# GinZhu/RDST

Hardware: AMD Instinct MI355X
Metric: SR patches/sec fwd+bwd, RDST-E1 x4 64->256 (higher is better)
Workload: dtype bf16; 1 GPU; RDST-E1 x4 (RDST_E1_OASIS_example_SRx4.ini), 1x64x64 LR patches -> 256x256, step = fwd + L1 + bwd + flat-bucket grad all-reduce + Adam; global_batch=32, per_gpu_batch=32, parallelism=dp1, hip_graph=True, grad_bucket_bytes=17859844

## Files before the change

### rdst_amd/csrc/lnlin3_mfma.hip

```cpp
#include "linear.h"
#include "lds_dma.h"
#include "mfma.h"
#include "wattn_hd.h"
#include <stdlib.h>

#ifndef LB3_LOADW_SHAPE
#define LB3_LOADW_SHAPE(K, N) (((K) == 60 && (N) == 180) || ((K) == 90 && (N) == 270) || ((K) == 120 && (N) == 120))
#endif
#ifndef LB3_ABL
#define LB3_ABL 0
#endif

#ifdef LB3_STAMPS
constexpr bool LB3_TICKS = true;
#else
constexpr bool LB3_TICKS = false;
#endif
constexpr const char* LB3_LEGEND = "stash fetch barrier compute finish - - -";

namespace {
using namespace wahd;
using MM = Mma<bf16>;

struct LB3Args {
  const bf16* X; int64_t ldx; const float* stats; const float* lnw; const float* W;
  const bf16* dY; int64_t lddy; bf16* dX; int64_t lddx; const bf16* Acc; int64_t ldacc;
  const bf16* Acc2; int64_t ldacc2;
  float* slab; int64_t slab_stride;
  int64_t M; int64_t ntiles; int tiles_per_wg;
};

template <int K_, int N_>
struct LB3 {
  static constexpr int K = K_, N = N_;
  static constexpr int NCT = (K + 1 + 31) / 32, NW = (N + 31) / 32, KN = (N + 15) / 16;
  static constexpr bool WIDE = N >= 180;
  static constexpr int TN = WIDE ? 3 : 1;
  static constexpr int TC = (K == 120 && N == 360) ? 2 : WIDE ? 1 : NCT;
  static_assert(NW % TN == 0 && NCT % TC == 0, "blocking");
  static constexpr int NGN = NW / TN, NGC = NCT / TC, NWG = NGN * NGC;
  static constexpr int NDG = NCT;
  static constexpr int NWV = NWG + NDG, NT = 64 * NWV;
  static constexpr int PKX = (K * 2 + 15) / 16, PKY = (N * 2 + 15) / 16;
  static constexpr int NY = 32 * PKY, NX = 32 * PKX;
  static constexpr bool LOADW = LB3_LOADW_SHAPE(K_, N_);
  static constexpr bool SPLITR = WIDE || LOADW;
  static constexpr int NTW = SPLITR ? 64 * NWG : NT, NTD = SPLITR ? 64 * NDG : NT;
  static constexpr int cdiv(int a, int b) { return (a + b - 1) / b; }
  static constexpr bool ACC_BY_W = K == 120 && N == 360;
  static constexpr int W_SY = cdiv(NY, NTW), W_SX = cdiv(NX, NTW), W_SA = (WIDE && !ACC_BY_W && !LOADW) ? 0 : cdiv(NX, NTW);
  static constexpr int D_SY = SPLITR ? 0 : W_SY, D_SX = SPLITR ? 0 : W_SX, D_SA = (ACC_BY_W || LOADW) ? 0 : cdiv(NX, NTD);
  static constexpr int CP = 32 * NCT;
  static constexpr int LDX = NCT == 4 ? 336 : CP * 2 + 16;
  static constexpr int LDY = lds_plane_stride(32 * NW);
  static constexpr int OFF_AC = 32 * LDX, OFF_DY = 64 * LDX, OFF_SM = OFF_DY + 32 * LDY, BUF = OFF_SM + 128;
  static constexpr int OFF_RED = 2 * BUF;
  static constexpr int SMEM = OFF_RED + 2 * NCT * 256;
  static constexpr int PERCU0 = 12 / NWV < 1 ? 1 : 12 / NWV;
  static constexpr int PERCU1 = WIDE ? 1 : PERCU0 > 2 ? 2 : PERCU0;
  static constexpr int PERCU = PERCU1 * SMEM > 160 * 1024 ? 1 : PERCU1;
  static constexpr int WPS = (NWV * PERCU + 3) / 4;
};

template <class CF, bool LN, int SY, int SX, int SA>
struct LB3Loader {
  static constexpr int NS = SY + SX + SA;
  int meta[NS > 0 ? NS : 1];
  u32x4_a4 rd[NS > 0 ? NS : 1];
  u32x4_a4 rd2[SA > 0 ? SA : 1];
  float2 rst[SX > 0 ? SX : 1];
  static __device__ __forceinline__ int kind(int u) { return u < SY ? 0 : u < SY + SX ? 1 : 2; }
  __device__ __forceinline__ void setup(int tid_r, int ntr, bool has_acc) {
#pragma unroll
    for (int u = 0; u < NS; ++u) {
      const int kd = kind(u);
      const int idx = tid_r + ntr * (kd == 0 ? u : kd == 1 ? u - SY : u - SY - SX);
      const int per = kd == 0 ? CF::PKY : CF::PKX, rowbytes = kd == 0 ? CF::N * 2 : CF::K * 2;
      const bool on = idx < 32 * per && (kd != 2 || has_acc);
      const int row = on ? idx / per : 0, chk = on ? idx - row * per : 0;
      int o = chk * 16;
      if (o + 16 > rowbytes) o = rowbytes - 16;
      meta[u] = o | (row << 16) | ((on ? 1 : 0) << 24) | (((o & 15) == 0 ? 1 : 0) << 28);
    }
  }
  __device__ __forceinline__ void fetch(const LB3Args& p, int64_t tile) {
    const uint32_t Mu = (uint32_t)p.M;
#pragma unroll
    for (int u = 0; u < NS; ++u) {
      const int kd = kind(u);
      uint32_t row = (uint32_t)(tile * 32) + (uint32_t)((meta[u] >> 16) & 31);
      row = row < Mu ? row : Mu - 1;
      const char* base = reinterpret_cast<const char*>(kd == 0 ? p.dY : kd == 1 ? p.X : (p.Acc ? p.Acc : p.X));
      const uint32_t ldb = (uint32_t)((kd == 0 ? p.lddy : kd == 1 ? p.ldx : p.ldacc) * 2);
      rd[u] = *reinterpret_cast<const u32x4_a4*>(base + (size_t)(row * ldb + (uint32_t)(meta[u] & 0xffff)));
      if (kd == 2 && p.Acc2)
        rd2[u - SY - SX] = *reinterpret_cast<const u32x4_a4*>(reinterpret_cast<const char*>(p.Acc2) +
                                                              (size_t)(row * (uint32_t)(p.ldacc2 * 2) + (uint32_t)(meta[u] & 0xffff)));
      if (LN && kd == 1) rst[u - SY] = *reinterpret_cast<const float2*>(p.stats + 2 * (size_t)row);
    }
  }
  __device__ __forceinline__ void stash(const LB3Args& p, int64_t tile, char* buf) {
    const uint32_t Mu = (uint32_t)p.M;
#pragma unroll
    for (int u = 0; u < NS; ++u) {
      const int kd = kind(u);
      if (!((meta[u] >> 24) & 1)) continue;
      const int mrow = (meta[u] >> 16) & 31;
      const bool valid = (uint32_t)(tile * 32) + (uint32_t)mrow < Mu;
      Pack16 v;
      v.w[0] = valid ? rd[u].x : 0u; v.w[1] = valid ? rd[u].y : 0u; v.w[2] = valid ? rd[u].z : 0u; v.w[3] = valid ? rd[u].w : 0u;
      if (kd == 2 && p.Acc2) {
        const u32x4_a4 a = rd[u], b2 = rd2[u - SY - SX];
        const bool h1 = p.Acc != nullptr;
        float f[8];
        f[0] = bf16lo(b2.x) + (h1 ? bf16lo(a.x) : 0.f); f[1] = bf16hi(b2.x) + (h1 ? bf16hi(a.x) : 0.f);
        f[2] = bf16lo(b2.y) + (h1 ? bf16lo(a.y) : 0.f); f[3] = bf16hi(b2.y) + (h1 ? bf16hi(a.y) : 0.f);
        f[4] = bf16lo(b2.z) + (h1 ? bf16lo(a.z) : 0.f); f[5] = bf16hi(b2.z) + (h1 ? bf16hi(a.z) : 0.f);
        f[6] = bf16lo(b2.w) + (h1 ? bf16lo(a.w) : 0.f); f[7] = bf16hi(b2.w) + (h1 ? bf16hi(a.w) : 0.f);
#pragma unroll
        for (int e = 0; e < 8; ++e) f[e] = valid ? f[e] : 0.f;
        v = MM::pack(f);
      }
      if (LN && kd == 1) {
        const float2 st2 = rst[u - SY];
        float f[8];
        f[0] = bf16lo(rd[u].x); f[1] = bf16hi(rd[u].x); f[2] = bf16lo(rd[u].y); f[3] = bf16hi(rd[u].y);
        f[4] = bf16lo(rd[u].z); f[5] = bf16hi(rd[u].z); f[6] = bf16lo(rd[u].w); f[7] = bf16hi(rd[u].w);
#pragma unroll
        for (int e = 0; e < 8; ++e) f[e] = valid ? (f[e] - st2.x) * st2.y : 0.f;
        v = MM::pack(f);
        if ((meta[u] & 0xffff) == 0) reinterpret_cast<float*>(buf + CF::OFF_SM)[mrow] = st2.y;
      }
      int mt = meta[u];
      asm volatile("" : "+v"(mt));
      const int lrow = (mt >> 16) & 31, lo = mt & 0xffff;
      char* dst = buf + (kd == 0 ? CF::OFF_DY + lrow * CF::LDY : (kd == 2 ? CF::OFF_AC : 0) + lrow * CF::LDX) + lo;
      if ((meta[u] >> 28) & 1) *reinterpret_cast<Pack16*>(dst) = v;
      else {
        uint32_t* d = reinterpret_cast<uint32_t*>(dst);
        d[0] = v.w[0]; d[1] = v.w[1]; d[2] = v.w[2]; d[3] = v.w[3];
      }
    }
  }
};

template <int K, int N, bool LN>
__global__ void __launch_bounds__((LB3<K, N>::NT), (LB3<K, N>::WPS)) lnlin3_bwd_kernel(const LB3Args p) {
  extern __shared__ __attribute__((aligned(16))) char smem[];
  using CF = LB3<K, N>;
  constexpr int NCT = CF::NCT, NW = CF::NW, KN = CF::KN, TN = CF::TN, TC = CF::TC, NGC = CF::NGC, NWG = CF::NWG, NT = CF::NT;
  constexpr int LDX = CF::LDX, LDY = CF::LDY;
  const int tid = threadIdx.x, lane = tid & 63, wave = __builtin_amdgcn_readfirstlane(tid >> 6), r = lane & 31, hh = lane >> 5;
  const bool has_acc = p.Acc != nullptr || p.Acc2 != nullptr;

  if (!(LB3_ABL & 16)) lds_zero16(smem, CF::SMEM, tid, NT);
  __syncthreads();
  if (tid < 64) *reinterpret_cast<uint16_t*>(smem + (tid >> 5) * CF::BUF + (tid & 31) * LDX + K * 2) = 0x3f80;

  const int q = (lane & 15) >> 2, pp = lane & 3, gq1 = (lane >> 4) & 1;
  const int trc = (16 * gq1 + 4 * pp) * 2;
  const int tro_y = CF::OFF_DY + (8 * hh + q) * LDY + trc;
  const int tro_x = (8 * hh + q) * LDX + trc;

  const bool is_wg = wave < NWG;
  const int gn = wave / NGC, gc = wave - gn * NGC;
  const int dct = wave - NWG;

  const int64_t t0 = (int64_t)blockIdx.x * p.tiles_per_wg;
  const int64_t t1 = t0 + p.tiles_per_wg < p.ntiles ? t0 + p.tiles_per_wg : p.ntiles;
  __syncthreads();

  if (is_wg) {
    LB3Loader<CF, LN, CF::W_SY, CF::W_SX, CF::W_SA> ld;
    ld.setup(tid, CF::NTW, has_acc);
    if (t0 < t1) ld.fetch(p, t0);
    f32x16 G[TN][TC];
#pragma unroll
    for (int i = 0; i < TN; ++i)
#pragma unroll
      for (int j = 0; j < TC; ++j)
#pragma unroll
        for (int v = 0; v < 16; ++v) G[i][j][v] = 0.f;
    int b = 0;
    WaveTicks<LB3_TICKS> wt;
    for (int64_t tile = t0; tile < t1; ++tile, b ^= 1) {
      char* buf = smem + b * CF::BUF;
      ld.stash(p, tile, buf);
      wt.add(0);
      ld.fetch(p, tile + 1 < t1 ? tile + 1 : tile);
      wt.add(1);
      __syncthreads();
      wt.add(2);
#pragma unroll
      for (int s = 0; s < 2; ++s) {
        Pack16 ya[TN], xb[TC];
#pragma unroll
        for (int i = 0; i < TN; ++i) {
          const lds_cp yp = (lds_cp)(buf + tro_y + 16 * s * LDY) + (gn * TN + i) * 64;
          ya[i] = lds_tr_pack(yp, yp + 4 * LDY);
        }
#pragma unroll
        for (int j = 0; j < TC; ++j) {
          const lds_cp xp = (lds_cp)(buf + tro_x + 16 * s * LDX) + (gc * TC + j) * 64;
          xb[j] = lds_tr_pack(xp, xp + 4 * LDX);
        }
#pragma unroll
        for (int i = 0; i < TN; ++i)
#pragma unroll
          for (int j = 0; j < TC; ++j) {
#if !(LB3_ABL & 1)
            MM::mma(G[i][j], ya[i], xb[j]);
#else
            G[i][j][0] += __uint_as_float(ya[i].w[0] ^ xb[j].w[0]);
#endif
          }
      }
      wt.add(3);
    }
    wt.print(wave, lane, "wgrad", LB3_LEGEND);
    if (LN) __syncthreads();
    uint2* my = reinterpret_cast<uint2*>(p.slab) + (int64_t)blockIdx.x * p.slab_stride;
#pragma unroll
    for (int i = 0; i < TN; ++i)
#pragma unroll
      for (int j = 0; j < TC; ++j) {
        const int c = 32 * (gc * TC + j) + r;
#pragma unroll
        for (int g4 = 0; g4 < 4; ++g4) {
          const int n0 = 32 * (gn * TN + i) + 8 * g4 + 4 * hh;
          if (n0 < N && c <= K && !(LB3_ABL & 8))
            my[(int64_t)(n0 >> 2) * (K + 1) + c] =
                make_uint2(pack_bf16x2(G[i][j][4 * g4], G[i][j][4 * g4 + 1]), pack_bf16x2(G[i][j][4 * g4 + 2], G[i][j][4 * g4 + 3]));
        }
      }
    return;
  }

  LB3Loader<CF, LN, CF::D_SY, CF::D_SX, CF::D_SA> ld;
  ld.setup(CF::SPLITR ? tid - 64 * NWG : tid, CF::NTD, has_acc);
  if (t0 < t1) ld.fetch(p, t0);
  Pack16 wf[KN];
  {
    const int c = 32 * dct + r;
    const int cc = c < K ? c : K - 1;
    const float gm = (c < K) ? (LN ? p.lnw[cc] : 1.0f) : 0.f;
#pragma unroll
    for (int ks = 0; ks < KN; ++ks) {
      float f[8];
#pragma unroll
      for (int e = 0; e < 8; ++e) {
        const int n = 16 * ks + 8 * hh + e;
#if LB3_ABL & 4
        const float w = 0.01f * (float)(n + cc);
#else
        const float w = p.W[(size_t)(n < N ? n : N - 1) * K + cc];
#endif
        f[e] = n < N ? w * gm : 0.f;
      }
      wf[ks] = MM::pack(f);
    }
  }
  constexpr float invK = 1.0f / (float)K;
  float* red = reinterpret_cast<float*>(smem + CF::OFF_RED);
  f32x16 dx;
  u32x2_t xs[4], as[4];
  float rstd = 0.f;
  int64_t prow = -1;
  auto finish = [&](int pb) {
    float s1 = 0.f, s2 = 0.f;
    if (LN) {
#pragma unroll
      for (int w = 0; w < NCT; ++w) {
        const float2 v = *reinterpret_cast<const float2*>(red + ((pb * NCT + w) * 32 + r) * 2);
        s1 += v.x; s2 += v.y;
      }
      s1 *= invK; s2 *= invK;
    }
    float o[16];
#pragma unroll
    for (int g4 = 0; g4 < 4; ++g4) {
      const float xh[4] = {bf16lo(xs[g4].x), bf16hi(xs[g4].x), bf16lo(xs[g4].y), bf16hi(xs[g4].y)};
      const float ac[4] = {bf16lo(as[g4].x), bf16hi(as[g4].x), bf16lo(as[g4].y), bf16hi(as[g4].y)};
#pragma unroll
      for (int e = 0; e < 4; ++e) o[4 * g4 + e] = LN ? fmaf(rstd, dx[4 * g4 + e] - s1 - xh[e] * s2, ac[e]) : dx[4 * g4 + e] + ac[e];
    }
    if (prow < p.M) {
      bf16* drow = p.dX + prow * p.lddx;
#pragma unroll
      for (int gp2 = 0; gp2 < 2; ++gp2) {
        float c8[8];
#pragma unroll
        for (int e = 0; e < 4; ++e) {
          const auto sw = __builtin_amdgcn_permlane32_swap(__float_as_uint(o[8 * gp2 + e]), __float_as_uint(o[8 * gp2 + 4 + e]), false, false);
          c8[e] = __uint_as_float(sw[0]);
          c8[4 + e] = __uint_as_float(sw[1]);
        }
        const int cb = 32 * dct + 8 * (2 * gp2 + hh);
        if (cb + 8 <= K) {
          u32x4_a4 u;
          u.x = pack_bf16x2(c8[0], c8[1]); u.y = pack_bf16x2(c8[2], c8[3]);
          u.z = pack_bf16x2(c8[4], c8[5]); u.w = pack_bf16x2(c8[6], c8[7]);
          *reinterpret_cast<u32x4_a4*>(drow + cb) = u;
        } else {
#pragma unroll
          for (int e = 0; e < 8; ++e)
            if (cb + e < K) drow[cb + e] = __float2bfloat16(c8[e]);
        }
      }
    }
  };
  int b = 0;
  WaveTicks<LB3_TICKS> wt;
  for (int64_t tile = t0; tile < t1; ++tile, b ^= 1) {
    char* buf = smem + b * CF::BUF;
    ld.stash(p, tile, buf);
    wt.add(0);
    ld.fetch(p, tile + 1 < t1 ? tile + 1 : tile);
    wt.add(1);
    __syncthreads();
    wt.add(2);
    if (LN && prow >= 0) finish(b ^ 1);
    wt.add(4);
    const lds_cp yrow = (lds_cp)(buf + CF::OFF_DY + r * LDY + hh * 16);
#pragma unroll
    for (int v = 0; v < 16; ++v) dx[v] = 0.f;
    if constexpr (KN > 12) {
#pragma unroll
      for (int ks = 0; ks < KN; ++ks) {
#if !(LB3_ABL & 2)
        MM::mma(dx, wf[ks], lds_pack(yrow + 32 * ks));
#else
        dx[0] += __uint_as_float(lds_pack(yrow + 32 * ks).w[0]);
#endif
      }
    } else {
      f32x16 d2;
#pragma unroll
      for (int v = 0; v < 16; ++v) d2[v] = 0.f;
#pragma unroll
      for (int ks = 0; ks < KN; ++ks) {
        const Pack16 yb = lds_pack(yrow + 32 * ks);
        if (ks & 1) MM::mma(d2, wf[ks], yb);
        else MM::mma(dx, wf[ks], yb);
      }
#pragma unroll
      for (int v = 0; v < 16; ++v) dx[v] += d2[v];
    }
    const lds_cp xrow = (lds_cp)(buf + r * LDX) + (32 * dct + 4 * hh) * 2;
#pragma unroll
    for (int g4 = 0; g4 < 4; ++g4) {
      xs[g4] = *reinterpret_cast<const LDS_AS u32x2_t*>(xrow + 16 * g4);
      as[g4] = *reinterpret_cast<const LDS_AS u32x2_t*>(xrow + CF::OFF_AC + 16 * g4);
    }
    prow = tile * 32 + r;
    if (LN) {
      rstd = reinterpret_cast<const float*>(buf + CF::OFF_SM)[r];
      float s1 = 0.f, s2 = 0.f;
#pragma unroll
      for (int g4 = 0; g4 < 4; ++g4) {
        const float xh[4] = {bf16lo(xs[g4].x), bf16hi(xs[g4].x), bf16lo(xs[g4].y), bf16hi(xs[g4].y)};
#pragma unroll
        for (int e = 0; e < 4; ++e) {
          s1 += dx[4 * g4 + e];
          s2 = fmaf(dx[4 * g4 + e], xh[e], s2);
        }
      }
      s1 = half_swap_sum(s1);
      s2 = half_swap_sum(s2);
      if (hh == 0) *reinterpret_cast<float2*>(red + ((b * NCT + dct) * 32 + r) * 2) = make_float2(s1, s2);
    } else {
      wt.add(3);
      finish(b);
      wt.add(4);
    }
    wt.add(3);
  }
  wt.print(wave, lane, "dgrad", LB3_LEGEND);
  if (LN) {
    __syncthreads();
    if (prow >= 0) finish(b ^ 1);
  }
}

template <int K, int N, bool LN>
int lb3_launch(LB3Args& p, const WsSlab& slab, int* grid_out, hipStream_t st) {
  using CF = LB3<K, N>;
  auto kern = lnlin3_bwd_kernel<K, N, LN>;
  static int percu_env = -1;
  if (percu_env < 0) { const char* e = rdst_dbg_getenv("RDST_LB3_PERCU"); percu_env = e ? atoi(e) : 0; }
  int per_cu = CF::PERCU;
  if (percu_env > 0 && percu_env < per_cu) per_cu = percu_env;
  const int64_t grid = rdst_tile_grid(p.ntiles, slab.cap((int64_t)kCUs * per_cu, 2 * p.slab_stride), &p.tiles_per_wg);
  if (int rc = rdst_slab_fits(slab, grid, 2 * p.slab_stride, "lnlin3_bwd")) return rc;
  *grid_out = (int)grid;
  return rdst_launch(kern, dim3((unsigned)grid), dim3(CF::NT), CF::SMEM, st, "lnlin3_bwd", p);
}

}

int lnlin3_bwd_bf16(const bf16* X, int64_t ldx, const float* ln_w, const float* stats, const float* Wt, const bf16* dY,
                    int64_t lddy, bf16* dX, int64_t lddx, const bf16* acc, int64_t ldacc, const bf16* acc2, int64_t ldacc2,
                    const WsSlab& slab, int64_t slab_stride, int64_t M, int K, int N, int* grid_out, hipStream_t st) {
  static int off = -1;
  if (off < 0) { const char* e = rdst_dbg_getenv("RDST_LB3_OFF"); off = e ? atoi(e) : 0; }
  if (off) return RDST_ENOTSUP;
  const bool ln = ln_w != nullptr;
  LB3Args p{};
  p.X = X; p.ldx = ldx; p.stats = stats; p.lnw = ln_w; p.W = Wt; p.dY = dY; p.lddy = lddy; p.dX = dX; p.lddx = lddx;
  p.Acc = acc; p.ldacc = ldacc; p.Acc2 = acc2; p.ldacc2 = ldacc2; p.slab = slab.p; p.slab_stride = slab_stride; p.M = M;
  p.ntiles = (M + 31) / 32;
#define RDST_LB3(KK, NN, LL) if (K == KK && N == NN && ln == LL) return lb3_launch<KK, NN, LL>(p, slab, grid_out, st);
  RDST_LB3(60, 180, true) RDST_LB3(90, 270, true) RDST_LB3(120, 360, true)
  RDST_LB3(60, 30, true) RDST_LB3(90, 30, true) RDST_LB3(120, 30, true)
  RDST_LB3(60, 60, false) RDST_LB3(90, 90, false) RDST_LB3(120, 120, false)
#undef RDST_LB3
  return RDST_ENOTSUP;
}
```

Baseline: 1943 patches/s.

## Add LDS-DMA ring-buffer prefetch path for square plain Linear backward

For square Linear backward shapes without LayerNorm or accumulators (K==N in 60/90/120), replaces the register-staged double-buffered loader with a multi-buffer ring (default 4 slots) fed by direct global-to-LDS DMA, issued by the weight-grad waves several tiles ahead. Synchronisation is done with vmcnt waits, and a small patch step writes the ones column and zero tails. This aims to hide load latency and remove the register round-trip and LDS zeroing. The cost is more LDS per workgroup and reliance on exact vmcnt accounting, with an environment switch to disable the path.

```diff
diff --git a/rdst_amd/csrc/lnlin3_mfma.hip b/rdst_amd/csrc/lnlin3_mfma.hip
--- a/rdst_amd/csrc/lnlin3_mfma.hip
+++ b/rdst_amd/csrc/lnlin3_mfma.hip
@@ -3,9 +3,13 @@
 #include "mfma.h"
 #include "wattn_hd.h"
 #include <stdlib.h>
+#include <type_traits>
 
 #ifndef LB3_LOADW_SHAPE
 #define LB3_LOADW_SHAPE(K, N) (((K) == 60 && (N) == 180) || ((K) == 90 && (N) == 270) || ((K) == 120 && (N) == 120))
+#endif
+#ifndef LB3_RING_NBUF
+#define LB3_RING_NBUF(K) 4
 #endif
 #ifndef LB3_ABL
 #define LB3_ABL 0
@@ -60,7 +64,71 @@
   static constexpr int PERCU1 = WIDE ? 1 : PERCU0 > 2 ? 2 : PERCU0;
   static constexpr int PERCU = PERCU1 * SMEM > 160 * 1024 ? 1 : PERCU1;
   static constexpr int WPS = (NWV * PERCU + 3) / 4;
+  static constexpr int NBUF = LB3_RING_NBUF(K_);
+  static constexpr int RSX = LDX / 16, RSY = LDY / 16;
+  static constexpr int RPX = cdiv(32 * RSX, 64), RPY = cdiv(32 * RSY, 64), RNP = RPX + RPY;
+  static constexpr int ROFF_DY = RPX * 1024, RBUF = RNP * 1024, RSMEM = NBUF * RBUF;
+  static constexpr int RCNT = cdiv(RNP, NWG);
 };
+
+#ifndef LB3_RING_SHAPE
+#define LB3_RING_SHAPE(K, N) ((K) == (N) && ((K) == 60 || (K) == 90 || (K) == 120))
+#endif
+
+template <class CF>
+struct LB3Ring {
+  static constexpr int ROWB = CF::K * 2, TAILCH = ROWB / 16, TAILB = ROWB % 16;
+  static_assert(CF::RNP >= CF::NWG && CF::RCNT * (CF::NBUF - 2) < 64, "vmcnt is a 6-bit counter");
+  static_assert(CF::RSX > TAILCH && (TAILB == 0 || CF::RSY > TAILCH), "the ones column lies inside the row");
+  uint32_t rel[CF::RCNT];
+  int fix;
+  int wv;
+  __device__ __forceinline__ int piece(int i) const {
+    const int q = wv + CF::NWG * i;
+    return q < CF::RNP ? q : q - CF::NWG;
+  }
+  __device__ __forceinline__ void setup(int wave, int lane) {
+    wv = wave;
+    fix = 0;
+#pragma unroll
+    for (int i = 0; i < CF::RCNT; ++i) {
+      const int q = piece(i);
+      const bool isx = q < CF::RPX;
+      const int s = (isx ? q : q - CF::RPX) * 64 + lane, sl = isx ? CF::RSX : CF::RSY;
+      const int row = s / sl, ch = s - row * sl;
+      rel[i] = (row < 32 && ch * 16 < ROWB) ? (uint32_t)(row * ROWB + ch * 16) : 0x80000000u;
+      if (row < 32 && ch == TAILCH && (isx || TAILB != 0)) fix |= (isx ? 2 : 1) << (2 * i);
+    }
+  }
+  __device__ __forceinline__ void issue(const u32x4s_t& rsx, const u32x4s_t& rsy, uint32_t lds0, int64_t tile, int b) const {
+    const uint32_t tb = (uint32_t)tile * (uint32_t)(32 * ROWB);
+#pragma unroll
+    for (int i = 0; i < CF::RCNT; ++i) {
+      const int q = piece(i);
+      lds_dma16(q < CF::RPX ? rsx : rsy, __builtin_amdgcn_readfirstlane(lds0 + (uint32_t)(b * CF::RBUF + q * 1024)), (int)(tb + rel[i]));
+    }
+  }
+  __device__ __forceinline__ void patch(char* buf, int lane) const {
+#pragma unroll
+    for (int i = 0; i < CF::RCNT; ++i) {
+      const int code = (fix >> (2 * i)) & 3;
+      if (code) {
+        uint32_t* d = reinterpret_cast<uint32_t*>(buf + piece(i) * 1024 + lane * 16 + TAILB);
+        d[0] = code == 2 ? 0x3f80u : 0u;
+#pragma unroll
+        for (int e = 1; e < (16 - TAILB) / 4; ++e) d[e] = 0u;
+      }
+    }
+  }
+};
+struct LB3NoLoader {};
+
+template <int CNT, int D>
+__device__ __forceinline__ void lb3_wait_tiles(int64_t younger) {
+  if constexpr (D == 0) wait_vmcnt<0>();
+  else if (younger >= D) wait_vmcnt<CNT * D>();
+  else lb3_wait_tiles<CNT, D - 1>(younger);
+}
 
 template <class CF, bool LN, int SY, int SX, int SA>
 struct LB3Loader {
@@ -144,22 +212,26 @@
   }
 };
 
-template <int K, int N, bool LN>
+template <int K, int N, bool LN, bool RING = false>
 __global__ void __launch_bounds__((LB3<K, N>::NT), (LB3<K, N>::WPS)) lnlin3_bwd_kernel(const LB3Args p) {
   extern __shared__ __attribute__((aligned(16))) char smem[];
   using CF = LB3<K, N>;
+  static_assert(!RING || (!LN && K == N), "the ring takes plain Linear shapes with x and dY rows of one length");
   constexpr int NCT = CF::NCT, NW = CF::NW, KN = CF::KN, TN = CF::TN, TC = CF::TC, NGC = CF::NGC, NWG = CF::NWG, NT = CF::NT;
   constexpr int LDX = CF::LDX, LDY = CF::LDY;
+  constexpr int BUFB = RING ? CF::RBUF : CF::BUF, OFF_DY = RING ? CF::ROFF_DY : CF::OFF_DY, NBUF = RING ? CF::NBUF : 2;
   const int tid = threadIdx.x, lane = tid & 63, wave = __builtin_amdgcn_readfirstlane(tid >> 6), r = lane & 31, hh = lane >> 5;
   const bool has_acc = p.Acc != nullptr || p.Acc2 != nullptr;
 
-  if (!(LB3_ABL & 16)) lds_zero16(smem, CF::SMEM, tid, NT);
-  __syncthreads();
-  if (tid < 64) *reinterpret_cast<uint16_t*>(smem + (tid >> 5) * CF::BUF + (tid & 31) * LDX + K * 2) = 0x3f80;
+  if constexpr (!RING) {
+    if (!(LB3_ABL & 16)) lds_zero16(smem, CF::SMEM, tid, NT);
+    __syncthreads();
+    if (tid < 64) *reinterpret_cast<uint16_t*>(smem + (tid >> 5) * CF::BUF + (tid & 31) * LDX + K * 2) = 0x3f80;
+  }
 
   const int q = (lane & 15) >> 2, pp = lane & 3, gq1 = (lane >> 4) & 1;
   const int trc = (16 * gq1 + 4 * pp) * 2;
-  const int tro_y = CF::OFF_DY + (8 * hh + q) * LDY + trc;
+  const int tro_y = OFF_DY + (8 * hh + q) * LDY + trc;
   const int tro_x = (8 * hh + q) * LDX + trc;
 
   const bool is_wg = wave < NWG;
@@ -168,12 +240,24 @@
 
   const int64_t t0 = (int64_t)blockIdx.x * p.tiles_per_wg;
   const int64_t t1 = t0 + p.tiles_per_wg < p.ntiles ? t0 + p.tiles_per_wg : p.ntiles;
-  __syncthreads();
+  if constexpr (!RING) __syncthreads();
 
   if (is_wg) {
-    LB3Loader<CF, LN, CF::W_SY, CF::W_SX, CF::W_SA> ld;
-    ld.setup(tid, CF::NTW, has_acc);
-    if (t0 < t1) ld.fetch(p, t0);
+    std::conditional_t<RING, LB3Ring<CF>, LB3Loader<CF, LN, CF::W_SY, CF::W_SX, CF::W_SA>> ld;
+    u32x4s_t rsx, rsy;
+    uint32_t lds0 = 0;
+    if constexpr (RING) {
+      rsx = dma_rsrc(p.X, (uint32_t)(p.M * (K * 2)));
+      rsy = dma_rsrc(p.dY, (uint32_t)(p.M * (N * 2)));
+      lds0 = lds_base(smem);
+      ld.setup(wave, lane);
+#pragma unroll
+      for (int a = 0; a < NBUF - 1; ++a)
+        if (t0 + a < t1) ld.issue(rsx, rsy, lds0, t0 + a, a);
+    } else {
+      ld.setup(tid, CF::NTW, has_acc);
+      if (t0 < t1) ld.fetch(p, t0);
+    }
     f32x16 G[TN][TC];
 #pragma unroll
     for (int i = 0; i < TN; ++i)
@@ -183,14 +267,24 @@
         for (int v = 0; v < 16; ++v) G[i][j][v] = 0.f;
     int b = 0;
     WaveTicks<LB3_TICKS> wt;
-    for (int64_t tile = t0; tile < t1; ++tile, b ^= 1) {
-      char* buf = smem + b * CF::BUF;
-      ld.stash(p, tile, buf);
-      wt.add(0);
-      ld.fetch(p, tile + 1 < t1 ? tile + 1 : tile);
-      wt.add(1);
-      __syncthreads();
-      wt.add(2);
+    for (int64_t tile = t0; tile < t1; ++tile, b = (RING ? (b + 1 == NBUF ? 0 : b + 1) : b ^ 1)) {
+      char* buf = smem + b * BUFB;
+      if constexpr (RING) {
+        lb3_wait_tiles<CF::RCNT, NBUF - 2>(t1 - 1 - tile);
+        ld.patch(buf, lane);
+        wt.add(0);
+        __syncthreads();
+        wt.add(2);
+        if (tile + (NBUF - 1) < t1) ld.issue(rsx, rsy, lds0, tile + (NBUF - 1), b == 0 ? NBUF - 1 : b - 1);
+        wt.add(1);
+      } else {
+        ld.stash(p, tile, buf);
+        wt.add(0);
+        ld.fetch(p, tile + 1 < t1 ? tile + 1 : tile);
+        wt.add(1);
+        __syncthreads();
+        wt.add(2);
+      }
 #pragma unroll
       for (int s = 0; s < 2; ++s) {
         Pack16 ya[TN], xb[TC];
@@ -236,9 +330,11 @@
     return;
   }
 
-  LB3Loader<CF, LN, CF::D_SY, CF::D_SX, CF::D_SA> ld;
-  ld.setup(CF::SPLITR ? tid - 64 * NWG : tid, CF::NTD, has_acc);
-  if (t0 < t1) ld.fetch(p, t0);
+  std::conditional_t<RING, LB3NoLoader, LB3Loader<CF, LN, CF::D_SY, CF::D_SX, CF::D_SA>> ld;
+  if constexpr (!RING) {
+    ld.setup(CF::SPLITR ? tid - 64 * NWG : tid, CF::NTD, has_acc);
+    if (t0 < t1) ld.fetch(p, t0);
+  }
   Pack16 wf[KN];
   {
     const int c = 32 * dct + r;
@@ -311,17 +407,19 @@
   };
   int b = 0;
   WaveTicks<LB3_TICKS> wt;
-  for (int64_t tile = t0; tile < t1; ++tile, b ^= 1) {
-    char* buf = smem + b * CF::BUF;
-    ld.stash(p, tile, buf);
-    wt.add(0);
-    ld.fetch(p, tile + 1 < t1 ? tile + 1 : tile);
-    wt.add(1);
+  for (int64_t tile = t0; tile < t1; ++tile, b = (RING ? (b + 1 == NBUF ? 0 : b + 1) : b ^ 1)) {
+    char* buf = smem + b * BUFB;
+    if constexpr (!RING) {
+      ld.stash(p, tile, buf);
+      wt.add(0);
+      ld.fetch(p, tile + 1 < t1 ? tile + 1 : tile);
+      wt.add(1);
+    }
     __syncthreads();
     wt.add(2);
     if (LN && prow >= 0) finish(b ^ 1);
     wt.add(4);
-    const lds_cp yrow = (lds_cp)(buf + CF::OFF_DY + r * LDY + hh * 16);
+    const lds_cp yrow = (lds_cp)(buf + OFF_DY + r * LDY + hh * 16);
 #pragma unroll
     for (int v = 0; v < 16; ++v) dx[v] = 0.f;
     if constexpr (KN > 12) {
@@ -350,7 +448,8 @@
 #pragma unroll
     for (int g4 = 0; g4 < 4; ++g4) {
       xs[g4] = *reinterpret_cast<const LDS_AS u32x2_t*>(xrow + 16 * g4);
-      as[g4] = *reinterpret_cast<const LDS_AS u32x2_t*>(xrow + CF::OFF_AC + 16 * g4);
+      if constexpr (RING) as[g4] = u32x2_t{0u, 0u};
+      else as[g4] = *reinterpret_cast<const LDS_AS u32x2_t*>(xrow + CF::OFF_AC + 16 * g4);
     }
     prow = tile * 32 + r;
     if (LN) {
@@ -382,10 +481,22 @@
   }
 }
 
-template <int K, int N, bool LN>
+template <int K, int N>
+bool lb3_ring_ok(const LB3Args& p) {
+  static int off = -1;
+  if (off < 0) { const char* e = rdst_dbg_getenv("RDST_LB3_RING_OFF"); off = e ? atoi(e) : 0; }
+  return !off && !p.Acc && !p.Acc2 && p.ldx == K && p.lddy == N && (((uintptr_t)p.X | (uintptr_t)p.dY) & 15) == 0 &&
+         (uint64_t)p.M * (uint64_t)(K * 2) < (1ull << 31);
+}
+
+template <int K, int N, bool LN, bool RING = false>
 int lb3_launch(LB3Args& p, const WsSlab& slab, int* grid_out, hipStream_t st) {
   using CF = LB3<K, N>;
-  auto kern = lnlin3_bwd_kernel<K, N, LN>;
+  if constexpr (!RING && !LN && LB3_RING_SHAPE(K, N))
+    if (lb3_ring_ok<K, N>(p)) return lb3_launch<K, N, LN, true>(p, slab, grid_out, st);
+  auto kern = lnlin3_bwd_kernel<K, N, LN, RING>;
+  constexpr int SMEM = RING ? CF::RSMEM : CF::SMEM;
+  static_assert(SMEM * CF::PERCU <= 160 * 1024, "LDS of the workgroups that share a CU");
   static int percu_env = -1;
   if (percu_env < 0) { const char* e = rdst_dbg_getenv("RDST_LB3_PERCU"); percu_env = e ? atoi(e) : 0; }
   int per_cu = CF::PERCU;
@@ -393,7 +504,7 @@
   const int64_t grid = rdst_tile_grid(p.ntiles, slab.cap((int64_t)kCUs * per_cu, 2 * p.slab_stride), &p.tiles_per_wg);
   if (int rc = rdst_slab_fits(slab, grid, 2 * p.slab_stride, "lnlin3_bwd")) return rc;
   *grid_out = (int)grid;
-  return rdst_launch(kern, dim3((unsigned)grid), dim3(CF::NT), CF::SMEM, st, "lnlin3_bwd", p);
+  return rdst_launch(kern, dim3((unsigned)grid), dim3(CF::NT), SMEM, st, "lnlin3_bwd", p);
 }
 
 }
```

After: 1952 patches/s (median of 6 runs). About the same (+0.5%).
